# KeyuWu-CS/MonoHair

Hardware: AMD Instinct MI355X
Metric: PMVO iterations/sec (60x1080p views, 256^3 volume) (higher is better)
Workload: dtype f32

## Files before the change

### monohair_amd/csrc/pmvo_search.hip

```cpp
#include "mh_search_common.h"
#include "../../include/mh_pmvo_lab.h"

__device__ __forceinline__ void mh_sample_next(const float *__restrict__ cam, float X0, float X1, float X2,
                                               float ori_r, float ori_c, float Hf, float Wf, float off, float &S0,
                                               float &S1, float &S2, int forms) {
    alignas(16) float rec[16];
    mh_sample_rank(cam, X0, X1, X2, ori_r, ori_c, Hf, Wf, rec, forms);
    mh_sample_item(reinterpret_cast<const float4 *>(rec), off, S0, S1, S2);
}

__device__ __forceinline__ float mh_one_minus_abs(float x) {
    float r;
    asm("v_sub_f32_e64 %0, 1.0, |%1|" : "=v"(r) : "v"(x));
    return r;
}

template <int K, int T>
__global__ __launch_bounds__(T) void mh_search_kernel(MhViews vw, const float *__restrict__ offs, int S, int nrank,
                                                      int rank_step, const float *__restrict__ pts, int N, int P1,
                                                      float thr, const float *__restrict__ ori_c,
                                                      const int32_t *__restrict__ base_idx,
                                                      const float *__restrict__ base_val,
                                                      const float4 *__restrict__ taps, float *__restrict__ line_ori,
                                                      float *__restrict__ min_loss, uint8_t *__restrict__ high_conf,
                                                      float *__restrict__ best_sample, int32_t *__restrict__ best_rank,
                                                      int32_t *__restrict__ best_s, MhRule rule) {
    __shared__ float s_loss[MH_MAX_ITEMS];
    __shared__ uint8_t s_pos[MH_MAX_ITEMS];
    __shared__ float s_rl[MH_MAX_RANKS];
    __shared__ int s_ri[MH_MAX_RANKS];
    __shared__ int s_rh[MH_MAX_RANKS];

    const int n = blockIdx.x, tid = threadIdx.x;
    const int nitems = nrank * S;
    const int V = vw.V;
    const float Hf = (float)vw.H, Wf = (float)vw.W;
    const float P0 = pts[3 * n], P1x = pts[3 * n + 1], P2 = pts[3 * n + 2];

    float X0[K], X1[K], X2[K];
    MhCascV num[K], den[K];
    int cnt[K];
    const int tail_from = mh_tail_from(rule, n, S);
#pragma unroll
    for (int j = 0; j < K; ++j) {
        int it = j * T + tid;
        it = it < nitems ? it : 0;
        const int r = it / S, s = it - r * S;
        const int b = min(max(base_idx[(size_t)(r * rank_step) * N + n], 0), V - 1);
        const float2 oc = reinterpret_cast<const float2 *>(ori_c)[(size_t)b * N + n];
        mh_sample_next(vw.cams + b * MH_CAM_STRIDE, P0, P1x, P2, oc.x, oc.y, Hf, Wf, offs[s], X0[j], X1[j], X2[j],
                       mh_group_forms(rule, r, V, b, S));
        num[j] = den[j] = MhCascV{0.0f, 0.0f, 0.0f};
        cnt[j] = 0;
    }

    for (int v = 0; v < V; ++v) {
        if (v > 0 && (v & 15) == 0) {
#pragma unroll
            for (int j = 0; j < K; ++j) {
                mh_cascv_flush(num[j], v);
                mh_cascv_flush(den[j], v);
            }
        }
        const float4 *__restrict__ rec = taps + ((size_t)v * N + n) * P1;
        const float4 hdr = rec[0];
        if (hdr.y == -1.0f) continue;
        const int ntap = __float_as_int(hdr.x);
        const float *__restrict__ cam = vw.cams + v * MH_CAM_STRIDE;
        const float4 t0 = rec[1];
        {
            float dx[K], dy[K], ml[K], bc[K];
#pragma unroll
            for (int j = 0; j < K; ++j) {
                float row, col;
                mh_pixel_of(cam, X0[j], X1[j], X2[j], Hf, Wf, row, col);
                mh_unit2(row - hdr.z, col - hdr.w, dx[j], dy[j]);
                const float cs = t0.x * dx[j] + t0.y * dy[j];
                ml[j] = 1.0f - __builtin_fabsf(cs);
                bc[j] = t0.z;
            }
            for (int t = 1; t < ntap; ++t) {
                const float4 tp = rec[1 + t];
#pragma unroll
                for (int j = 0; j < K; ++j) {
                    const float cs = tp.x * dx[j] + tp.y * dy[j];
                    const float l = 1.0f - __builtin_fabsf(cs);
                    const bool upd = l < ml[j];
                    ml[j] = upd ? l : ml[j];
                    bc[j] = upd ? tp.z : bc[j];
                }
            }
#pragma unroll
            for (int j = 0; j < K; ++j) {
                const float w = bc[j];
                num[j].a0 = num[j].a0 + ml[j] * w;
                den[j].a0 = den[j].a0 + w;
                cnt[j] += (w > 0.0f) ? 1 : 0;
            }
        }
    }

#pragma unroll
    for (int j = 0; j < K; ++j) {
        const int it = j * T + tid;
        if (it < nitems) {
            float dn = mh_cascv_done(den[j]);
            float nm = mh_cascv_done(num[j]);
            int cn = cnt[j];
            if (it - (it / S) * S >= tail_from)
                mh_tail_item_sums(vw.cams, V, Hf, Wf, taps + (size_t)n * P1, (size_t)N * P1, nullptr, N, X0[j], X1[j], X2[j],
                                  nm, dn, cn);
            const float ratio = dn / (float)cn;
            s_pos[it] = (ratio > thr) ? 1 : 0;
            s_loss[it] = nm / dn;
        }
    }
    const bool all_nan = mh_point_pixel_not_finite(vw, P0, P1x, P2, N, tid, T);

    const int wave = tid >> 6, lane = tid & 63, nwaves = T >> 6;
    for (int r = wave; r < nrank; r += nwaves) {
        int npos = 0;
        for (int s0 = 0; s0 < S; s0 += MH_WAVE) {
            const int s = s0 + lane;
            npos += __popcll(__ballot(s < S && s_pos[r * S + s]));
        }
        const bool low = npos < 5;
        float bl = 0.0f;
        int bi = 0x7fffffff;
        for (int s = lane; s < S; s += MH_WAVE) {
            float l = all_nan ? __builtin_nanf("") : s_loss[r * S + s];
            if (!low && !s_pos[r * S + s]) l = 1.0f;
            if (bi == 0x7fffffff || mh_min_better(l, s, bl, bi)) {
                bl = l;
                bi = s;
            }
        }
#pragma unroll
        for (int o = 32; o > 0; o >>= 1) {
            const float ol = __shfl_xor(bl, o);
            const int oi = __shfl_xor(bi, o);
            if (oi != 0x7fffffff && (bi == 0x7fffffff || mh_min_better(ol, oi, bl, bi))) {
                bl = ol;
                bi = oi;
            }
        }
        if (lane == 0) {
            s_rl[r] = bl;
            s_ri[r] = bi;
            s_rh[r] = s_pos[r * S + bi];
        }
    }
    __syncthreads();

    if (tid == 0) {
        const float Hf = (float)vw.H, Wf = (float)vw.W;
        float ml = s_rl[0];
        int br = 0, bs = s_ri[0], hc = s_rh[0];
        for (int r = 1; r < nrank; ++r) {
            const float l = s_rl[r];
            if ((l < ml) && (base_val[(size_t)(r * rank_step) * N + n] > 0.0f)) {
                ml = l;
                br = r;
                bs = s_ri[r];
                hc = s_rh[r];
            }
        }
        const int b = min(max(base_idx[(size_t)(br * rank_step) * N + n], 0), V - 1);
        const float2 oc = reinterpret_cast<const float2 *>(ori_c)[(size_t)b * N + n];
        float B0, B1, B2;
        mh_sample_next(vw.cams + b * MH_CAM_STRIDE, P0, P1x, P2, oc.x, oc.y, Hf, Wf, offs[bs], B0, B1, B2,
                       mh_group_forms(rule, br, V, b, S));
        const float d0 = B0 - P0, d1 = B1 - P1x, d2 = B2 - P2;
        float s2 = d0 * d0;
        s2 = mh_fma(d1, d1, s2);
        s2 = mh_fma(d2, d2, s2);
        const float nrm = __builtin_sqrtf(s2);
        line_ori[3 * n] = d0 / nrm;
        line_ori[3 * n + 1] = d1 / nrm;
        line_ori[3 * n + 2] = d2 / nrm;
        min_loss[n] = ml;
        high_conf[n] = (uint8_t)hc;
        if (best_sample) {
            best_sample[3 * n] = B0;
            best_sample[3 * n + 1] = B1;
            best_sample[3 * n + 2] = B2;
        }
        if (best_rank) best_rank[n] = br;
        if (best_s) best_s[n] = bs;
    }
}

__device__ __forceinline__ float mh_vmul(float a, float b) {
    float r;
    asm("v_mul_f32_e32 %0, %1, %2" : "=v"(r) : "v"(a), "v"(b));
    return r;
}
__device__ __forceinline__ float mh_vadd(float a, float b) {
    float r;
    asm("v_add_f32_e32 %0, %1, %2" : "=v"(r) : "v"(a), "v"(b));
    return r;
}

template <int KA>
__device__ __forceinline__ void mh_tap_update(float (&ML)[KA], float (&BC)[KA], const float (&l)[KA], float cf) {
    if constexpr (KA == 4) {
        unsigned long long m0, m1, m2, m3;
        asm("v_cmp_lt_f32_e64 %[m0], %[l0], %[a0]\n\t"
            "v_cmp_lt_f32_e64 %[m1], %[l1], %[a1]\n\t"
            "v_cmp_lt_f32_e64 %[m2], %[l2], %[a2]\n\t"
            "v_cmp_lt_f32_e64 %[m3], %[l3], %[a3]\n\t"
            "v_cndmask_b32_e64 %[a0], %[a0], %[l0], %[m0]\n\t"
            "v_cndmask_b32_e64 %[a1], %[a1], %[l1], %[m1]\n\t"
            "v_cndmask_b32_e64 %[a2], %[a2], %[l2], %[m2]\n\t"
            "v_cndmask_b32_e64 %[a3], %[a3], %[l3], %[m3]\n\t"
            "v_cndmask_b32_e64 %[b0], %[b0], %[cf], %[m0]\n\t"
            "v_cndmask_b32_e64 %[b1], %[b1], %[cf], %[m1]\n\t"
            "v_cndmask_b32_e64 %[b2], %[b2], %[cf], %[m2]\n\t"
            "v_cndmask_b32_e64 %[b3], %[b3], %[cf], %[m3]"
            : [a0] "+v"(ML[0]), [a1] "+v"(ML[1]), [a2] "+v"(ML[2]), [a3] "+v"(ML[3]), [b0] "+v"(BC[0]),
              [b1] "+v"(BC[1]), [b2] "+v"(BC[2]), [b3] "+v"(BC[3]), [m0] "=&s"(m0), [m1] "=&s"(m1), [m2] "=&s"(m2),
              [m3] "=&s"(m3)
            : [l0] "v"(l[0]), [l1] "v"(l[1]), [l2] "v"(l[2]), [l3] "v"(l[3]), [cf] "v"(cf));
    } else if constexpr (KA == 3) {
        unsigned long long m0, m1, m2;
        asm("v_cmp_lt_f32_e64 %[m0], %[l0], %[a0]\n\t"
            "v_cmp_lt_f32_e64 %[m1], %[l1], %[a1]\n\t"
            "v_cmp_lt_f32_e64 %[m2], %[l2], %[a2]\n\t"
            "v_cndmask_b32_e64 %[a0], %[a0], %[l0], %[m0]\n\t"
            "v_cndmask_b32_e64 %[a1], %[a1], %[l1], %[m1]\n\t"
            "v_cndmask_b32_e64 %[a2], %[a2], %[l2], %[m2]\n\t"
            "v_cndmask_b32_e64 %[b0], %[b0], %[cf], %[m0]\n\t"
            "v_cndmask_b32_e64 %[b1], %[b1], %[cf], %[m1]\n\t"
            "v_cndmask_b32_e64 %[b2], %[b2], %[cf], %[m2]"
            : [a0] "+v"(ML[0]), [a1] "+v"(ML[1]), [a2] "+v"(ML[2]), [b0] "+v"(BC[0]), [b1] "+v"(BC[1]),
              [b2] "+v"(BC[2]), [m0] "=&s"(m0), [m1] "=&s"(m1), [m2] "=&s"(m2)
            : [l0] "v"(l[0]), [l1] "v"(l[1]), [l2] "v"(l[2]), [cf] "v"(cf));
    } else if constexpr (KA == 2) {
        unsigned long long m0, m1;
        asm("v_cmp_lt_f32_e64 %[m0], %[l0], %[a0]\n\t"
            "v_cmp_lt_f32_e64 %[m1], %[l1], %[a1]\n\t"
            "s_nop 0\n\t"
            "v_cndmask_b32_e64 %[a0], %[a0], %[l0], %[m0]\n\t"
            "v_cndmask_b32_e64 %[a1], %[a1], %[l1], %[m1]\n\t"
            "v_cndmask_b32_e64 %[b0], %[b0], %[cf], %[m0]\n\t"
            "v_cndmask_b32_e64 %[b1], %[b1], %[cf], %[m1]"
            : [a0] "+v"(ML[0]), [a1] "+v"(ML[1]), [b0] "+v"(BC[0]), [b1] "+v"(BC[1]), [m0] "=&s"(m0), [m1] "=&s"(m1)
            : [l0] "v"(l[0]), [l1] "v"(l[1]), [cf] "v"(cf));
    } else {
#pragma unroll
        for (int j = 0; j < KA; ++j) {
            const bool upd = l[j] < ML[j];
            ML[j] = upd ? l[j] : ML[j];
            BC[j] = upd ? cf : BC[j];
        }
    }
}

#define MH_KEY_C 1.00006103515625f
#define MH_KEY_E 6.103515625e-05f
#define MH_KEY_BAD 0xF0000000u
#ifndef MH_KEY_MIN_TAPS
#define MH_KEY_MIN_TAPS 10
#endif
#define MH_KEY_PAD 4
template <bool BIGP>
__device__ __forceinline__ int mh_key_walked(int c) {
    return (c - (BIGP ? 0 : 1) + MH_KEY_PAD - 1) & ~(MH_KEY_PAD - 1);
}
template <bool BIGP>
__device__ __forceinline__ int mh_key_staged(int c) {
    const int w = mh_key_walked<BIGP>(c);
    return w > c ? w : c;
}
__device__ unsigned long long mh_key_stats_dev[4];
extern "C" int mh_debug_key_stats(unsigned long long *out, int reset) {
    if (hipMemcpyFromSymbol(out, HIP_SYMBOL(mh_key_stats_dev), sizeof(unsigned long long) * 4) != hipSuccess) return -1;
    if (reset) {
        const unsigned long long z[4] = {0, 0, 0, 0};
        if (hipMemcpyToSymbol(HIP_SYMBOL(mh_key_stats_dev), z, sizeof(z)) != hipSuccess) return -1;
    }
    return 0;
}
#define MH_KEY_COUNT_ALWAYS(i) do { if ((tid & 63) == 0) atomicAdd(&mh_key_stats_dev[i], 1ull); } while (0)
#ifdef MH_KEY_STATS
#define MH_KEY_COUNT(i) MH_KEY_COUNT_ALWAYS(i)
#else
#define MH_KEY_COUNT(i) do { } while (0)
#endif
__device__ __forceinline__ unsigned mh_tap_key(float cs, int idx) {
    float t;
    unsigned k;
    asm("v_sub_f32_e64 %0, %2, |%1|" : "=v"(t) : "v"(cs), "s"(MH_KEY_C));
    asm("v_lshl_or_b32 %0, %1, 5, %2" : "=v"(k) : "v"(t), "s"(idx));
    return k;
}
__device__ __forceinline__ unsigned mh_min3u(unsigned a, unsigned b, unsigned c) {
    unsigned r;
    asm("v_min3_u32 %0, %1, %2, %3" : "=v"(r) : "v"(a), "v"(b), "v"(c));
    return r;
}

#include "mh_key_blocks.h"

#define MH_S3_GRP 4
#ifndef MH_S3_WAVES
#define MH_S3_WAVES 5
#endif
#ifndef MH_S3_WAVES_SELECT
#define MH_S3_WAVES_SELECT MH_S3_WAVES
#endif
#define MH_S3_CAP 1280

template <bool BIG>
struct MhCascS {
    float a0 = 0.0f, a1 = 0.0f, a2 = 0.0f;
    __device__ __forceinline__ void flush(int v) {
        a1 = a1 + a0;
        a0 = 0.0f;
        if constexpr (BIG) {
            if ((v & 0xF0) == 0) {
                a2 = a2 + a1;
                a1 = 0.0f;
            }
        }
    }
    __device__ __forceinline__ float done() const { return BIG ? (a0 + a1) + a2 : (a0 + a1); }
};

__device__ __forceinline__ int mh_wave_prefix_sum(int x) {
#define MH_DPP_ADD(CTRL, ROWS) x += __builtin_amdgcn_update_dpp(0, x, CTRL, ROWS, 0xF, false)
    MH_DPP_ADD(0x111, 0xF);
    MH_DPP_ADD(0x112, 0xF);
    MH_DPP_ADD(0x114, 0xF);
    MH_DPP_ADD(0x118, 0xF);
    MH_DPP_ADD(0x142, 0xA);
    MH_DPP_ADD(0x143, 0xC);
#undef MH_DPP_ADD
    return x;
}

__device__ const float4 mh_zero_tap = {0.0f, 0.0f, 0.0f, 0.0f};
__device__ __forceinline__ void mh_stage_list(const float4 *__restrict__ src, float4 *dst, int nrec, int nfill, int lane) {
    for (int i0 = 0; i0 < nfill; i0 += 64) {
        const int i = i0 + lane;
        if (i < nfill) {
            const float4 *g = (i < nrec) ? src + i : &mh_zero_tap;
            __builtin_amdgcn_global_load_lds((const __attribute__((address_space(1))) void *)g,
                                             (__attribute__((address_space(3))) void *)(dst + i0), 16, 0, 0);
        }
    }
}

template <bool KEYS, bool BIGP>
__device__ __forceinline__ int mh_list_records(int c) {
    return c ? ((KEYS && c > MH_KEY_MIN_TAPS) ? mh_key_staged<BIGP>(c) : c) + 1 : 0;
}
template <int T, bool KEYS>
__device__ __forceinline__ void mh_stage_batch(const float4 *__restrict__ taps, float4 *s_taps, int vb, int n, int N, int P1,
                                               int c, int len, int pre, int base, unsigned long long take, int lane, int wave) {
    const unsigned place = __builtin_amdgcn_mbcnt_hi((unsigned)(take >> 32), __builtin_amdgcn_mbcnt_lo((unsigned)take, 0u));
    unsigned long long m = take & __ballot((int)(place & (T / 64 - 1)) == wave);
    while (m) {
        const int b = (int)__builtin_ctzll(m);
        m &= m - 1;
        const int L = __builtin_amdgcn_readlane(len, b);
        const int off = __builtin_amdgcn_readlane(pre, b) - L - base;
        const int lr = KEYS ? __builtin_amdgcn_readlane(c, b) + 1 : L;
        mh_stage_list(taps + ((size_t)(vb + b) * N + n) * P1, s_taps + off, lr, L, lane);
    }
}

template <int KA, int T, bool BIGV, bool KEYS, bool BIGP>
__device__ __forceinline__ void mh_search_slices_lds(const MhViews &vw, const float *__restrict__ offs, int S,
                                                     int n, int N, int P1, float thr,
                                                     const float4 *__restrict__ taps, const uint8_t *__restrict__ vcnt,
                                                     int nact, int tid, float *s_loss, uint8_t *s_pos, float4 *s_taps,
                                                     const float4 *s_rank, int c_first, int pre_first) {
    constexpr int KN = KA > 0 ? KA : 1;
    constexpr int KM = KA;
    const int V = vw.V;
    const float Hf = (float)vw.H, Wf = (float)vw.W;
    float X0[KN], X1[KN], X2[KN];
    MhCascS<BIGV> num[KN], den[KN];
    int cnt[KN];
    if constexpr (KA > 0) {
        const unsigned inv = (1u << 20) / (unsigned)S + 1u;
#pragma unroll
        for (int j = 0; j < KA; ++j) {
            int it = j * T + tid;
            it = it < nact ? it : 0;
            const int r = (int)(((unsigned)it * inv) >> 20), s = it - r * S;
            mh_sample_item(s_rank + 4 * r, offs[s], X0[j], X1[j], X2[j]);
            num[j] = den[j] = MhCascS<BIGV>{};
            cnt[j] = 0;
        }
    }
    int nf = 16;
    auto flush_upto = [&](int v) {
        while (nf <= v) {
#pragma unroll
            for (int j = 0; j < KN; ++j) {
                num[j].flush(nf);
                den[j].flush(nf);
            }
            nf += 16;
        }
    };
    auto one_view = [&](int v, const float4 *rec, int ntap) {
        const float *__restrict__ cam = vw.cams + v * MH_CAM_STRIDE;
        const float4 hdr = rec[0];
        const float4 t0 = rec[1];
        float DX[KN], DY[KN], ML[KN], BC[KN];
#pragma unroll
        for (int jp = 0; jp < KA / 2; ++jp) {
            mh_v2f row, col, dx, dy;
            mh_pixel_of_fast2(cam, mh_v2f{X0[2 * jp], X0[2 * jp + 1]}, mh_v2f{X1[2 * jp], X1[2 * jp + 1]},
                              mh_v2f{X2[2 * jp], X2[2 * jp + 1]}, Hf, Wf, row, col);
            mh_unit2_fast2(row - mh_splat(hdr.z), col - mh_splat(hdr.w), dx, dy);
            DX[2 * jp] = dx.x;
            DX[2 * jp + 1] = dx.y;
            DY[2 * jp] = dy.x;
            DY[2 * jp + 1] = dy.y;
        }
        if constexpr (KA & 1) {
            mh_v2f row, col, dx, dy;
            mh_pixel_of_fast2(cam, mh_splat(X0[KA - 1]), mh_splat(X1[KA - 1]), mh_splat(X2[KA - 1]), Hf, Wf, row, col);
            mh_unit2_fast2(row - mh_splat(hdr.z), col - mh_splat(hdr.w), dx, dy);
            DX[KA - 1] = dx.x;
            DY[KA - 1] = dy.x;
        }
        constexpr int GRP = MH_S3_GRP;
        auto select_body = [&]() {
#pragma unroll
            for (int j = 0; j < KA; ++j) {
                ML[j] = mh_one_minus_abs(mh_vadd(mh_vmul(t0.x, DX[j]), mh_vmul(t0.y, DY[j])));
                BC[j] = t0.z;
            }
            auto process = [&](const float4 (&g)[GRP], int t) {
#pragma unroll
                for (int u = 0; u < GRP; ++u) {
                    if (t + u < ntap) {
                        const float4 tp = g[u];
                        float l[KN];
#pragma unroll
                        for (int j = 0; j < KA; ++j)
                            l[j] = mh_one_minus_abs(mh_vadd(mh_vmul(tp.x, DX[j]), mh_vmul(tp.y, DY[j])));
                        mh_tap_update<KN>(ML, BC, l, tp.z);
                    }
                }
            };
            float4 ga[GRP], gb[GRP];
#pragma unroll
            for (int u = 0; u < GRP; ++u) ga[u] = rec[2 + u];
            for (int t = 1; t < ntap;) {
#pragma unroll
                for (int u = 0; u < GRP; ++u) gb[u] = rec[1 + t + GRP + u];
                process(ga, t);
                t += GRP;
                if (t >= ntap) break;
#pragma unroll
                for (int u = 0; u < GRP; ++u) ga[u] = rec[1 + t + GRP + u];
                process(gb, t);
                t += GRP;
            }
        };
        __builtin_amdgcn_s_setprio(0);
        if constexpr (!KEYS) {
            select_body();
        } else {
            bool again = (ntap <= MH_KEY_MIN_TAPS) || !(t0.x == t0.x && t0.y == t0.y);
            MH_KEY_COUNT(0);
            if (again) MH_KEY_COUNT(1);
            if (!again) {
                const int ntp = mh_key_walked<BIGP>(ntap);
                unsigned ke[KN], ko[KN];
                const unsigned rec1 = (unsigned)(size_t)(const __attribute__((address_space(3))) float4 *)(rec + 1);
                auto process = [&](const float2 (&g)[GRP], int t) {
                    const int ib = (t & 63) >> 1;
                    static_assert(MH_KEY_PAD == 4 && GRP == 4, "the key block takes four taps");
                    if constexpr (KM > 0) mh_key_block4<KM, KN>(ke, ko, g, DX, DY, ib);
                };
                auto group = [&](int ta, int tb) {
                    const float2 *__restrict__ t2 = reinterpret_cast<const float2 *>(rec + 1);
                    float2 ga[GRP], gb[GRP];
#pragma unroll
                    for (int u = 0; u < GRP; ++u) ga[u] = t2[2 * (ta + u)];
                    if constexpr (BIGP || KM == 0) {
#pragma unroll
                        for (int j = 0; j < KN; ++j) ke[j] = ko[j] = 0xFFFFFFFFu;
                    } else {
                        const int is = ntap - 1;
                        const float2 ts = t2[2 * is];
                        const bool even = (is & 1) == 0;
#pragma unroll
                        for (int j = 0; j < KM; ++j) {
                            const unsigned k = mh_tap_key(mh_vadd(mh_vmul(ts.x, DX[j]), mh_vmul(ts.y, DY[j])), is >> 1);
                            ke[j] = even ? k : 0xFFFFFFFFu;
                            ko[j] = even ? 0xFFFFFFFFu : k;
                        }
                    }
                    for (int t = ta; t < tb;) {
#pragma unroll
                        for (int u = 0; u < GRP; ++u) gb[u] = t2[2 * (t + GRP + u)];
                        process(ga, t);
                        t += GRP;
                        if (t >= tb) break;
#pragma unroll
                        for (int u = 0; u < GRP; ++u) ga[u] = t2[2 * (t + GRP + u)];
                        process(gb, t);
                        t += GRP;
                    }
                };
                unsigned best[KN], badr[KN];
                auto winner = [&](int ta, bool first) {
#pragma unroll
                    for (int j = 0; j < KM; ++j) {
                        const bool odd = ko[j] < ke[j];
                        const unsigned kb = odd ? ko[j] : ke[j];
                        const unsigned ad = rec1 + 16u * (unsigned)ta + ((kb & 31u) << 5) + (odd ? 16u : 0u);
                        const bool take = first || kb < (best[j] & ~31u);
                        best[j] = take ? kb : best[j];
                        badr[j] = take ? ad : badr[j];
                    }
                };
                if constexpr (!BIGP) {
                    group(0, ntp);
                    winner(0, true);
                } else {
                    group(0, ntp < 64 ? ntp : 64);
                    winner(0, true);
                    for (int ta = 64; ta < ntp; ta += 64) {
                        group(ta, ntp < ta + 64 ? ntp : ta + 64);
                        winner(ta, false);
                    }
                }
                unsigned worst = best[0];
#pragma unroll
                for (int j = 1; j < KM; ++j) worst = max(worst, best[j]);
                const bool bad = worst >= MH_KEY_BAD;
#pragma unroll
                for (int j = 0; j < KM; ++j) {
                    BC[j] = *reinterpret_cast<const __attribute__((address_space(3))) float *>((size_t)(badr[j] + 8u));
                    ML[j] = __uint_as_float(__builtin_amdgcn_alignbit(7u, best[j], 5u)) - MH_KEY_E;
                }
                again = __ballot(bad) != 0ull;
                if (again) MH_KEY_COUNT_ALWAYS(2);
            }
            if (again) select_body();
        }
        __builtin_amdgcn_s_setprio(1);
#pragma unroll
        for (int j = 0; j < KA; ++j) {
            const float w = BC[j];
            num[j].a0 = num[j].a0 + ML[j] * w;
            den[j].a0 = den[j].a0 + w;
            cnt[j] += (w > 0.0f) ? 1 : 0;
        }
    };
    const int lane = tid & 63, wave = __builtin_amdgcn_readfirstlane(tid >> 6);
    for (int vb = 0; vb < V; vb += 64) {
        const int vv = vb + lane;
        const int c = vb == 0 ? c_first : ((vv < V) ? (int)vcnt[(size_t)vv * N + n] : 0);
        const int len = mh_list_records<KEYS, BIGP>(c);
        const int pre = vb == 0 ? pre_first : mh_wave_prefix_sum(len);
        bool staged = vb == 0;
        unsigned long long todo = __ballot(c != 0);
        int base = 0;
        while (todo) {
            const unsigned long long take = todo & __ballot(pre - base <= MH_S3_CAP);
            if (!staged) {
                mh_stage_batch<T, KEYS>(taps, s_taps, vb, n, N, P1, c, len, pre, base, take, lane, wave);
                __syncthreads();
            }
            staged = false;
            if constexpr (KA > 0) {
                unsigned long long m = take;
                while (m) {
                    const int b = (int)__builtin_ctzll(m);
                    m &= m - 1;
                    flush_upto(vb + b);
                    const int L = __builtin_amdgcn_readlane(len, b);
                    const int off = __builtin_amdgcn_readlane(pre, b) - L - base;
                    one_view(vb + b, s_taps + off, KEYS ? __builtin_amdgcn_readlane(c, b) : L - 1);
                }
            }
            __syncthreads();
            base = __builtin_amdgcn_readlane(pre, 63 - (int)__builtin_clzll(take));
            todo &= ~take;
        }
    }
    if constexpr (KA > 0) {
        flush_upto(V - 1);
#pragma unroll
        for (int j = 0; j < KA; ++j) {
            const int it = j * T + tid;
            if (it < nact) {
                const float dn = den[j].done();
                const float nm = num[j].done();
                const float ratio = dn / (float)cnt[j];
                s_pos[it] = (ratio > thr) ? 1 : 0;
                s_loss[it] = nm / dn;
            }
        }
    }
}

template <int T, bool BIGV, bool KEYS, bool BIGP>
__global__ __launch_bounds__(T) __attribute__((amdgpu_waves_per_eu(KEYS ? MH_S3_WAVES : MH_S3_WAVES_SELECT))) void mh_search3_kernel(MhViews vw, const float *__restrict__ offs, int S, int nrank,
                                                       int rank_step, const float *__restrict__ pts, int N, int P1,
                                                       float thr, const float *__restrict__ ori_c,
                                                       const int32_t *__restrict__ base_idx,
                                                       const float *__restrict__ base_val,
                                                       const float4 *__restrict__ taps,
                                                       const uint8_t *__restrict__ vcnt,
                                                       const int32_t *__restrict__ order, float *__restrict__ line_ori,
                                                       float *__restrict__ min_loss, uint8_t *__restrict__ high_conf,
                                                       float *__restrict__ best_sample, int32_t *__restrict__ best_rank,
                                                       int32_t *__restrict__ best_s, MhRule rule) {
    __shared__ float4 s_taps[MH_S3_CAP + 8];
    __shared__ float s_loss[MH_MAX_ITEMS];
    __shared__ uint8_t s_pos[MH_MAX_ITEMS];
    __shared__ float s_rl[MH_MAX_RANKS];
    __shared__ int s_ri[MH_MAX_RANKS];
    __shared__ int s_rh[MH_MAX_RANKS];
    __shared__ float4 s_rank[MH_MAX_RANKS * 4];
    __shared__ float s_bval[MH_MAX_RANKS];
    __shared__ int s_tail;

    __builtin_amdgcn_s_setprio(1);
    const int tid = threadIdx.x;
    const int n = order ? order[blockIdx.x] : (int)blockIdx.x;
    const float P0 = pts[3 * n], P1x = pts[3 * n + 1], P2 = pts[3 * n + 2];
    const int c_first = ((tid & 63) < vw.V) ? (int)vcnt[(size_t)(tid & 63) * N + n] : 0;
    const int len_first = mh_list_records<KEYS, BIGP>(c_first);
    const int pre_first = mh_wave_prefix_sum(len_first);
    mh_stage_batch<T, KEYS>(taps, s_taps, 0, n, N, P1, c_first, len_first, pre_first, 0,
                            __ballot(c_first != 0) & __ballot(pre_first <= MH_S3_CAP), tid & 63,
                            __builtin_amdgcn_readfirstlane(tid >> 6));
    if (tid == 64) s_tail = mh_tail_from(rule, n, S);
    if (tid < nrank) {
        const size_t ro = (size_t)(tid * rank_step) * N + n;
        s_bval[tid] = base_val[ro];
        const int b = min(max(base_idx[ro], 0), vw.V - 1);
        const float2 oc = reinterpret_cast<const float2 *>(ori_c)[(size_t)b * N + n];
        mh_sample_rank(vw.cams + b * MH_CAM_STRIDE, P0, P1x, P2, oc.x, oc.y, (float)vw.H, (float)vw.W,
                       reinterpret_cast<float *>(s_rank + 4 * tid), mh_group_forms(rule, tid, vw.V, b, S));
    }
    __syncthreads();
    int nvalid = 1;
    for (int r = 1; r < nrank; ++r)
        if (s_bval[r] > 0.0f) nvalid = r + 1;
    const int nact = nvalid * S;
    const int wave0 = tid & ~63;
    int ka = 0;
    for (int j = 0; j < 4; ++j) ka += (j * T + wave0 < nact) ? 1 : 0;
#define MH_S3_ARGS vw, offs, S, n, N, P1, thr, taps, vcnt, nact, tid, s_loss, s_pos, s_taps, s_rank, c_first, pre_first
    if (ka == 4) mh_search_slices_lds<4, T, BIGV, KEYS, BIGP>(MH_S3_ARGS);
    else if (ka == 3) mh_search_slices_lds<3, T, BIGV, KEYS, BIGP>(MH_S3_ARGS);
    else if (ka == 2) mh_search_slices_lds<2, T, BIGV, KEYS, BIGP>(MH_S3_ARGS);
    else if (ka == 1) mh_search_slices_lds<1, T, BIGV, KEYS, BIGP>(MH_S3_ARGS);
    else mh_search_slices_lds<0, T, BIGV, KEYS, BIGP>(MH_S3_ARGS);
#undef MH_S3_ARGS
    __syncthreads();
    if (s_tail < S) {
        const int tail_from = s_tail;
        for (int it = tid; it < nact; it += T) {
            const int r = it / S, s = it - r * S;
            if (s < tail_from) continue;
            float X0, X1, X2, nm, dn;
            int cnt;
            mh_sample_item(s_rank + 4 * r, offs[s], X0, X1, X2);
            mh_tail_item_sums(vw.cams, vw.V, (float)vw.H, (float)vw.W, taps + (size_t)n * P1, (size_t)N * P1, vcnt + n, N, X0, X1,
                              X2, nm, dn, cnt);
            s_pos[it] = (dn / (float)cnt > thr) ? 1 : 0;
            s_loss[it] = nm / dn;
        }
        __syncthreads();
    }

    const bool all_nan = mh_point_pixel_not_finite(vw, P0, P1x, P2, N, tid, T);
    const int wave = tid >> 6, lane = tid & 63, nwaves = T >> 6;
    for (int r = wave; r < nvalid; r += nwaves) {
        int npos = 0;
        for (int s0 = 0; s0 < S; s0 += MH_WAVE) {
            const int s = s0 + lane;
            npos += __popcll(__ballot(s < S && s_pos[r * S + s]));
        }
        const bool low = npos < 5;
        float bl = 0.0f;
        int bi = 0x7fffffff;
        for (int s = lane; s < S; s += MH_WAVE) {
            float l = all_nan ? __builtin_nanf("") : s_loss[r * S + s];
            if (!low && !s_pos[r * S + s]) l = 1.0f;
            if (bi == 0x7fffffff || mh_min_better(l, s, bl, bi)) {
                bl = l;
                bi = s;
            }
        }
#pragma unroll
        for (int o = 32; o > 0; o >>= 1) {
            const float ol = __shfl_xor(bl, o);
            const int oi = __shfl_xor(bi, o);
            if (oi != 0x7fffffff && (bi == 0x7fffffff || mh_min_better(ol, oi, bl, bi))) {
                bl = ol;
                bi = oi;
            }
        }
        if (lane == 0) {
            s_rl[r] = bl;
            s_ri[r] = bi;
            s_rh[r] = s_pos[r * S + bi];
        }
    }
    __syncthreads();

    if (tid == 0) {
        float ml = s_rl[0];
        int br = 0, bs = s_ri[0], hc = s_rh[0];
        for (int r = 1; r < nvalid; ++r) {
            const float l = s_rl[r];
            if ((l < ml) && (s_bval[r] > 0.0f)) {
                ml = l;
                br = r;
                bs = s_ri[r];
                hc = s_rh[r];
            }
        }
        float B0, B1, B2;
        mh_sample_item(s_rank + 4 * br, offs[bs], B0, B1, B2);
        const float d0 = B0 - P0, d1 = B1 - P1x, d2 = B2 - P2;
        float s2 = d0 * d0;
        s2 = mh_fma(d1, d1, s2);
        s2 = mh_fma(d2, d2, s2);
        const float nrm = __builtin_sqrtf(s2);
        line_ori[3 * n] = d0 / nrm;
        line_ori[3 * n + 1] = d1 / nrm;
        line_ori[3 * n + 2] = d2 / nrm;
        min_loss[n] = ml;
        high_conf[n] = (uint8_t)hc;
        if (best_sample) {
            best_sample[3 * n] = B0;
            best_sample[3 * n + 1] = B1;
            best_sample[3 * n + 2] = B2;
        }
        if (best_rank) best_rank[n] = br;
        if (best_s) best_s[n] = bs;
    }
}

__global__ __launch_bounds__(256) void mh_search_work_kernel(const uint8_t *__restrict__ cnt, int V, int N, int P1,
                                                             const float *__restrict__ base_val, int nrank,
                                                             int rank_step, int S, int T, int32_t *__restrict__ order,
                                                             int tail_n0) {
    const int wave = threadIdx.x >> 6, lane = threadIdx.x & 63;
    const int n = blockIdx.x * 4 + wave;
    if (n >= N) return;
    int nt = 0;
    for (int v = lane; v < V; v += MH_WAVE) nt += cnt[(size_t)v * N + n];
#pragma unroll
    for (int o = 32; o > 0; o >>= 1) nt += __shfl_xor(nt, o);
    const bool usable = lane > 0 && lane < nrank && base_val[(size_t)(lane * rank_step) * N + n] > 0.0f;
    const unsigned long long m = __ballot(usable);
    const int nvalid = m ? (64 - __builtin_clzll(m)) : 1;
    if (lane == 0) order[n] = n >= tail_n0 ? 0 : mh_work_class(nt, nvalid, V, P1, S, T);
}

__global__ __launch_bounds__(256) void mh_group_sizes_kernel(const int32_t *__restrict__ base_idx, int N, int V,
                                                             int rank_step, int32_t *__restrict__ gcnt) {
    extern __shared__ int s_g[];
    const int r = blockIdx.y, tid = threadIdx.x;
    for (int i = tid; i < V; i += 256) s_g[i] = 0;
    __syncthreads();
    const int n = blockIdx.x * 256 + tid;
    if (n < N) {
        const int b = base_idx[(size_t)(r * rank_step) * N + n];
        if (b >= 0 && b < V) atomicAdd(&s_g[b], 1);
    }
    __syncthreads();
    for (int i = tid; i < V; i += 256)
        if (s_g[i]) atomicAdd(&gcnt[(((int)blockIdx.x & (MH_GROUP_COPIES - 1)) * MH_GROUP_RANKS + r) * V + i], s_g[i]);
}

__global__ __launch_bounds__(1024) void mh_search_order_kernel(int N, int32_t *__restrict__ order) {
    __shared__ int s_hist[MH_ORDER_BUCKETS];
    __shared__ int s_part[1024 / 64];
    const int tid = threadIdx.x;
    s_hist[tid] = 0;
    __syncthreads();
    for (int n = tid; n < N; n += 1024) atomicAdd(&s_hist[order[n]], 1);
    __syncthreads();
    const int mine = s_hist[tid];
    int incl = mine;
#pragma unroll
    for (int o = 1; o < 64; o <<= 1) {
        const int x = __shfl_up(incl, o);
        if ((tid & 63) >= o) incl += x;
    }
    if ((tid & 63) == 63) s_part[tid >> 6] = incl;
    __syncthreads();
    int base = 0;
    for (int w = 0; w < (tid >> 6); ++w) base += s_part[w];
    __syncthreads();
    s_hist[tid] = base + incl - mine;
    __syncthreads();
    for (int n = tid; n < N; n += 1024) order[N + atomicAdd(&s_hist[order[n]], 1)] = n;
}

extern "C" int mh_launch_search(MhViews vw, const float *offs, int S, int nrank, int rank_step, const float *pts,
                                int N, int P1, float thr, const float *ori_c, const int32_t *base_idx,
                                const float *base_val, const float4 *taps, int32_t *order ,
                                const uint8_t *cnt ,
                                float *line_ori, float *min_loss, uint8_t *high_conf, float *best_sample,
                                int32_t *best_rank, int32_t *best_s, MhSearchPlan plan, int rule_mode, int fma_min_cols,
                                int sum_block, int32_t *gcnt ,
                                int groups_ready ,
                                hipStream_t st) {
    const int nitems = nrank * S;
    if (nitems > MH_MAX_ITEMS || nrank > MH_MAX_RANKS || nitems < 1) return -1;
    if (sum_block < 0) return -1;
    MhRule rule;
    rule.mode = rule_mode;
    rule.fma_min_cols = fma_min_cols;
    rule.gcnt = (rule_mode == 0) ? gcnt : nullptr;
    if (rule_mode == 0 && !gcnt) return -1;
    const long long cols = (long long)N * S;
    rule.tail_col0 = sum_block ? cols - cols % sum_block : cols;
    const bool portable = plan.portable || !cnt;
    if (rule.gcnt && !groups_ready && plan.part != MhSearchPlan::PART_KERNEL_ONLY) {
        if (hipMemsetAsync(gcnt, 0, sizeof(int32_t) * (size_t)MH_GROUP_COPIES * MH_GROUP_RANKS * vw.V, st) != hipSuccess) return -1;
        hipLaunchKernelGGL(mh_group_sizes_kernel, dim3((N + 255) / 256, nrank), dim3(256), sizeof(int) * (size_t)vw.V, st,
                           base_idx, N, vw.V, rank_step, gcnt);
    }
    if (!portable) {
        const int32_t *ord = nullptr;
        if (plan.order != MhSearchPlan::ORDER_NATURAL && order && N > 1) {
            if (plan.part != MhSearchPlan::PART_KERNEL_ONLY) {
                if (plan.order == MhSearchPlan::ORDER_BY_WORK)
                    hipLaunchKernelGGL(mh_search_work_kernel, dim3((N + 3) / 4), dim3(256), 0, st, cnt, vw.V, N, P1, base_val,
                                       nrank, rank_step, S, 256, order, (int)(rule.tail_col0 / S));
                hipLaunchKernelGGL(mh_search_order_kernel, dim3(1), dim3(1024), 0, st, N, order);
            }
            ord = order + N;
        }
        if (plan.part == MhSearchPlan::PART_PRE_ONLY) return (int)hipGetLastError();
#define MH_S3_LAUNCH(BIG, KEYS, BIGP)                                                                                   \
    hipLaunchKernelGGL((mh_search3_kernel<256, BIG, KEYS, BIGP>), dim3(N), dim3(256), 0, st, vw, offs, S, nrank, rank_step, \
                       pts, N, P1, thr, ori_c, base_idx, base_val, taps, cnt, ord, line_ori, min_loss, high_conf,       \
                       best_sample, best_rank, best_s, rule)
        const bool bigp = P1 - 1 > 64;
        if (vw.V > 256) {
            if (plan.select_body) MH_S3_LAUNCH(true, false, false);
            else if (bigp) MH_S3_LAUNCH(true, true, true);
            else MH_S3_LAUNCH(true, true, false);
        } else {
            if (plan.select_body) MH_S3_LAUNCH(false, false, false);
            else if (bigp) MH_S3_LAUNCH(false, true, true);
            else MH_S3_LAUNCH(false, true, false);
        }
#undef MH_S3_LAUNCH
    } else {
        hipLaunchKernelGGL((mh_search_kernel<4, 256>), dim3(N), dim3(256), 0, st, vw, offs, S, nrank, rank_step, pts, N, P1,
                           thr, ori_c, base_idx, base_val, taps, line_ori, min_loss, high_conf, best_sample, best_rank,
                           best_s, rule);
    }
    return (int)hipGetLastError();
}

extern "C" int mh_preload_pmvo_search() {
    hipFuncAttributes a;
    return (int)hipFuncGetAttributes(&a, reinterpret_cast<const void *>(&mh_search_order_kernel));
}
```

Baseline: 1713.

## Handle leftover search items with view-parallel pass in last wave

When the active item count leaves a small remainder (at most 16) past a multiple of 64, the last wave no longer gives each leftover item its own lane. Instead it spreads the leftover items across lanes per staged view, writes per-view (min-loss, weight) pairs to LDS, then reduces them per item in view order. This targets the under-filled tail wave, where most lanes sat idle while a few walked every view serially. As a smaller change, the per-lane `len` value is dropped and list lengths are recomputed from `c` after readlane. The cost is extra LDS, more template instantiations, and extra wavefront-scope fencing.

```diff
diff --git a/monohair_amd/csrc/pmvo_search.hip b/monohair_amd/csrc/pmvo_search.hip
--- a/monohair_amd/csrc/pmvo_search.hip
+++ b/monohair_amd/csrc/pmvo_search.hip
@@ -339,6 +339,12 @@
     return x;
 }
 
+__device__ __forceinline__ int mh_lane_now() {
+    int lane;
+    asm volatile("v_mbcnt_lo_u32_b32 %0, -1, 0\n\tv_mbcnt_hi_u32_b32 %0, -1, %0" : "=v"(lane));
+    return lane;
+}
+
 __device__ const float4 mh_zero_tap = {0.0f, 0.0f, 0.0f, 0.0f};
 __device__ __forceinline__ void mh_stage_list(const float4 *__restrict__ src, float4 *dst, int nrec, int nfill, int lane) {
     for (int i0 = 0; i0 < nfill; i0 += 64) {
@@ -355,27 +361,127 @@
 __device__ __forceinline__ int mh_list_records(int c) {
     return c ? ((KEYS && c > MH_KEY_MIN_TAPS) ? mh_key_staged<BIGP>(c) : c) + 1 : 0;
 }
-template <int T, bool KEYS>
+template <int T, bool KEYS, bool BIGP>
 __device__ __forceinline__ void mh_stage_batch(const float4 *__restrict__ taps, float4 *s_taps, int vb, int n, int N, int P1,
-                                               int c, int len, int pre, int base, unsigned long long take, int lane, int wave) {
+                                               int c, int pre, int base, unsigned long long take, int wave) {
+    const int lane = mh_lane_now();
     const unsigned place = __builtin_amdgcn_mbcnt_hi((unsigned)(take >> 32), __builtin_amdgcn_mbcnt_lo((unsigned)take, 0u));
     unsigned long long m = take & __ballot((int)(place & (T / 64 - 1)) == wave);
     while (m) {
         const int b = (int)__builtin_ctzll(m);
         m &= m - 1;
-        const int L = __builtin_amdgcn_readlane(len, b);
+        const int cb = __builtin_amdgcn_readlane(c, b);
+        const int L = mh_list_records<KEYS, BIGP>(cb);
         const int off = __builtin_amdgcn_readlane(pre, b) - L - base;
-        const int lr = KEYS ? __builtin_amdgcn_readlane(c, b) + 1 : L;
+        const int lr = cb + 1;
         mh_stage_list(taps + ((size_t)(vb + b) * N + n) * P1, s_taps + off, lr, L, lane);
     }
 }
 
-template <int KA, int T, bool BIGV, bool KEYS, bool BIGP>
+#define MH_S3_LEFT_MAX 16
+#define MH_S3_LEFT_PAIRS 544
+struct MhLeft {
+    float2 *pair;
+    unsigned *view;
+    unsigned long long *vis;
+};
+
+__device__ __forceinline__ void mh_left_batch(const float *__restrict__ cams, float Hf, float Wf, int V,
+                                                        const float *__restrict__ offs, int S, const float4 *s_rank,
+                                                        const float4 *s_taps, MhLeft lf, int nact, int L, int vb, int c,
+                                                        int len, int pre, int base, unsigned long long take) {
+    const int lane = mh_lane_now();
+    const unsigned place = __builtin_amdgcn_mbcnt_hi((unsigned)(take >> 32), __builtin_amdgcn_mbcnt_lo((unsigned)take, 0u));
+    if ((take >> lane) & 1ull) lf.view[place] = (unsigned)(pre - len - base) | ((unsigned)c << 11) | ((unsigned)lane << 18);
+    __builtin_amdgcn_fence(__ATOMIC_ACQ_REL, "wavefront");
+    const int nv = __popcll(take);
+    const int lg = L > 1 ? 32 - __builtin_clz((unsigned)(L - 1)) : 0;
+    const int i = lane & ((1 << lg) - 1);
+    const bool mine = i < L;
+    const int it = nact - L + (mine ? i : 0);
+    const int r = (int)(((unsigned)it * ((1u << 20) / (unsigned)S + 1u)) >> 20), s = it - r * S;
+    float X0, X1, X2;
+    mh_sample_item(s_rank + 4 * r, offs[s], X0, X1, X2);
+    for (int k0 = 0; k0 < nv; k0 += 64 >> lg) {
+        const int k = k0 + (lane >> lg);
+        const bool act = mine && k < nv;
+        const unsigned e = lf.view[act ? k : k0];
+        const int v = vb + (int)((e >> 18) & 63u);
+        const int ntap = act ? (int)((e >> 11) & 127u) : 0;
+        const float4 *rec = s_taps + (e & 2047u);
+        const float4 hdr = rec[0];
+        float row, col, dx, dy;
+        mh_pixel_of(cams + v * MH_CAM_STRIDE, X0, X1, X2, Hf, Wf, row, col);
+        mh_unit2(row - hdr.z, col - hdr.w, dx, dy);
+        const float4 t0 = rec[1];
+        float ml = 1.0f - __builtin_fabsf(t0.x * dx + t0.y * dy), bc = t0.z;
+        for (int t = 1; t < ntap; t += 4) {
+            float4 g[4];
+#pragma unroll
+            for (int u = 0; u < 4; ++u) g[u] = rec[1 + t + u];
+#pragma unroll
+            for (int u = 0; u < 4; ++u) {
+                const float l = 1.0f - __builtin_fabsf(g[u].x * dx + g[u].y * dy);
+                const bool upd = (t + u < ntap) && (l < ml);
+                ml = upd ? l : ml;
+                bc = upd ? g[u].z : bc;
+            }
+        }
+        if (act) lf.pair[i * V + v] = float2{ml, bc};
+    }
+}
+
+__device__ __forceinline__ void mh_left_sums(MhLeft lf, int V, int nact, int L, float thr, float *s_loss,
+                                                       uint8_t *s_pos) {
+    const int lane = mh_lane_now();
+    __builtin_amdgcn_fence(__ATOMIC_ACQ_REL, "wavefront");
+    if (lane >= L) return;
+    MhCascS<false> num, den;
+    int cnt = 0, nf = 16;
+    for (int vb = 0; vb < V; vb += 64) {
+        unsigned long long m = lf.vis[vb >> 6];
+        while (m) {
+            int v[4];
+            float2 e[4];
+#pragma unroll
+            for (int u = 0; u < 4; ++u) {
+                v[u] = m ? vb + (int)__builtin_ctzll(m) : -1;
+                m &= m - 1;
+                e[u] = lf.pair[lane * V + (v[u] < 0 ? 0 : v[u])];
+            }
+#pragma unroll
+            for (int u = 0; u < 4; ++u) {
+                if (v[u] < 0) break;
+                for (; nf <= v[u]; nf += 16) {
+                    num.flush(nf);
+                    den.flush(nf);
+                }
+                const float w = e[u].y;
+                num.a0 = num.a0 + e[u].x * w;
+                den.a0 = den.a0 + w;
+                cnt += (w > 0.0f) ? 1 : 0;
+            }
+        }
+    }
+    for (; nf <= V - 1; nf += 16) {
+        num.flush(nf);
+        den.flush(nf);
+    }
+    const int it = nact - L + lane;
+    const float dn = den.done();
+    const float nm = num.done();
+    const float ratio = dn / (float)cnt;
+    s_pos[it] = (ratio > thr) ? 1 : 0;
+    s_loss[it] = nm / dn;
+}
+
+template <int KA, int T, bool BIGV, bool KEYS, bool BIGP, bool LEFT = false>
 __device__ __forceinline__ void mh_search_slices_lds(const MhViews &vw, const float *__restrict__ offs, int S,
                                                      int n, int N, int P1, float thr,
                                                      const float4 *__restrict__ taps, const uint8_t *__restrict__ vcnt,
                                                      int nact, int tid, float *s_loss, uint8_t *s_pos, float4 *s_taps,
-                                                     const float4 *s_rank, int c_first, int pre_first) {
+                                                     const float4 *s_rank, int c_first, int pre_first, MhLeft lf,
+                                                     int left ) {
     constexpr int KN = KA > 0 ? KA : 1;
     constexpr int KM = KA;
     const int V = vw.V;
@@ -558,18 +664,23 @@
         }
     };
     const int lane = tid & 63, wave = __builtin_amdgcn_readfirstlane(tid >> 6);
+    int c = c_first, pre = pre_first;
     for (int vb = 0; vb < V; vb += 64) {
-        const int vv = vb + lane;
-        const int c = vb == 0 ? c_first : ((vv < V) ? (int)vcnt[(size_t)vv * N + n] : 0);
-        const int len = mh_list_records<KEYS, BIGP>(c);
-        const int pre = vb == 0 ? pre_first : mh_wave_prefix_sum(len);
+        if (vb) {
+            const int vv = vb + lane;
+            c = (vv < V) ? (int)vcnt[(size_t)vv * N + n] : 0;
+            pre = mh_wave_prefix_sum(mh_list_records<KEYS, BIGP>(c));
+        }
         bool staged = vb == 0;
         unsigned long long todo = __ballot(c != 0);
         int base = 0;
+        if constexpr (LEFT) {
+            if (left && lane == 0) lf.vis[vb >> 6] = todo;
+        }
         while (todo) {
             const unsigned long long take = todo & __ballot(pre - base <= MH_S3_CAP);
             if (!staged) {
-                mh_stage_batch<T, KEYS>(taps, s_taps, vb, n, N, P1, c, len, pre, base, take, lane, wave);
+                mh_stage_batch<T, KEYS, BIGP>(taps, s_taps, vb, n, N, P1, c, pre, base, take, wave);
                 __syncthreads();
             }
             staged = false;
@@ -579,10 +690,14 @@
                     const int b = (int)__builtin_ctzll(m);
                     m &= m - 1;
                     flush_upto(vb + b);
-                    const int L = __builtin_amdgcn_readlane(len, b);
+                    const int cb = __builtin_amdgcn_readlane(c, b);
+                    const int L = mh_list_records<KEYS, BIGP>(cb);
                     const int off = __builtin_amdgcn_readlane(pre, b) - L - base;
-                    one_view(vb + b, s_taps + off, KEYS ? __builtin_amdgcn_readlane(c, b) : L - 1);
+                    one_view(vb + b, s_taps + off, cb);
                 }
+            }
+            if constexpr (LEFT) {
+                if (left) mh_left_batch(vw.cams, Hf, Wf, V, offs, S, s_rank, s_taps, lf, nact, left, vb, c, mh_list_records<KEYS, BIGP>(c), pre, base, take);
             }
             __syncthreads();
             base = __builtin_amdgcn_readlane(pre, 63 - (int)__builtin_clzll(take));
@@ -602,6 +717,9 @@
                 s_loss[it] = nm / dn;
             }
         }
+    }
+    if constexpr (LEFT) {
+        if (left) mh_left_sums(lf, V, nact, left, thr, s_loss, s_pos);
     }
 }
 
@@ -626,6 +744,9 @@
     __shared__ float4 s_rank[MH_MAX_RANKS * 4];
     __shared__ float s_bval[MH_MAX_RANKS];
     __shared__ int s_tail;
+    __shared__ float2 s_left[BIGV ? 1 : MH_S3_LEFT_PAIRS];
+    __shared__ unsigned s_lview[BIGV ? 1 : 64];
+    __shared__ unsigned long long s_lvis[BIGV ? 1 : 4];
 
     __builtin_amdgcn_s_setprio(1);
     const int tid = threadIdx.x;
@@ -634,8 +755,8 @@
     const int c_first = ((tid & 63) < vw.V) ? (int)vcnt[(size_t)(tid & 63) * N + n] : 0;
     const int len_first = mh_list_records<KEYS, BIGP>(c_first);
     const int pre_first = mh_wave_prefix_sum(len_first);
-    mh_stage_batch<T, KEYS>(taps, s_taps, 0, n, N, P1, c_first, len_first, pre_first, 0,
-                            __ballot(c_first != 0) & __ballot(pre_first <= MH_S3_CAP), tid & 63,
+    mh_stage_batch<T, KEYS, BIGP>(taps, s_taps, 0, n, N, P1, c_first, pre_first, 0,
+                            __ballot(c_first != 0) & __ballot(pre_first <= MH_S3_CAP),
                             __builtin_amdgcn_readfirstlane(tid >> 6));
     if (tid == 64) s_tail = mh_tail_from(rule, n, S);
     if (tid < nrank) {
@@ -651,11 +772,21 @@
     for (int r = 1; r < nrank; ++r)
         if (s_bval[r] > 0.0f) nvalid = r + 1;
     const int nact = nvalid * S;
+    const int nrest = __builtin_amdgcn_readfirstlane(nact & 63);
+    const int nleft = (!BIGV && KEYS && nrest <= MH_S3_LEFT_MAX && nrest * vw.V <= MH_S3_LEFT_PAIRS) ? nrest : 0;
     const int wave0 = tid & ~63;
     int ka = 0;
-    for (int j = 0; j < 4; ++j) ka += (j * T + wave0 < nact) ? 1 : 0;
-#define MH_S3_ARGS vw, offs, S, n, N, P1, thr, taps, vcnt, nact, tid, s_loss, s_pos, s_taps, s_rank, c_first, pre_first
-    if (ka == 4) mh_search_slices_lds<4, T, BIGV, KEYS, BIGP>(MH_S3_ARGS);
+    for (int j = 0; j < 4; ++j) ka += (j * T + wave0 < nact - nleft) ? 1 : 0;
+    const MhLeft lf{s_left, s_lview, s_lvis};
+#define MH_S3_ARGS vw, offs, S, n, N, P1, thr, taps, vcnt, nact, tid, s_loss, s_pos, s_taps, s_rank, c_first, pre_first, lf, nleft
+    if (!BIGV && wave0 == T - 64 && nleft) {
+        if constexpr (!BIGV) {
+            if (ka == 3) mh_search_slices_lds<3, T, BIGV, KEYS, BIGP, true>(MH_S3_ARGS);
+            else if (ka == 2) mh_search_slices_lds<2, T, BIGV, KEYS, BIGP, true>(MH_S3_ARGS);
+            else if (ka == 1) mh_search_slices_lds<1, T, BIGV, KEYS, BIGP, true>(MH_S3_ARGS);
+            else mh_search_slices_lds<0, T, BIGV, KEYS, BIGP, true>(MH_S3_ARGS);
+        }
+    } else if (ka == 4) mh_search_slices_lds<4, T, BIGV, KEYS, BIGP>(MH_S3_ARGS);
     else if (ka == 3) mh_search_slices_lds<3, T, BIGV, KEYS, BIGP>(MH_S3_ARGS);
     else if (ka == 2) mh_search_slices_lds<2, T, BIGV, KEYS, BIGP>(MH_S3_ARGS);
     else if (ka == 1) mh_search_slices_lds<1, T, BIGV, KEYS, BIGP>(MH_S3_ARGS);
```

Measured after the change: 1755 (median of 6 runs). +2.5%, better.
